# otaviog/align3d

Hardware: AMD Instinct MI355X
Metric: ICP frame-pairs/sec (640x480, 3-lvl, 15 iters) (higher is better)
Workload: dtype f32; 1 GPU; ms3x15 x 64 pairs/GPU, distinct frames, 640x480, 3 lvl x 15 it, HBM-resident (configs[4] shard); pairs_per_gpu=64, global_pairs=64, levels=3, distinct_frames=True, ranks_in_collective=1, collective=none

## Files before the change

### align3d_amd/csrc/image_icp.hip

```cpp
#include <cstdlib>
#include <memory>

#include "icp_engine.hpp"

using namespace a3d;

namespace {

struct LevelDesc {
  const float* src_points;
  const uint8_t* src_mask;
  const uint8_t* src_intensities;
  const float* tgt_points;
  const float* tgt_normals;
  const uint8_t* tgt_mask;
  const float* imap;
  uint32_t src_n;
  uint32_t tw, th;
  float fx, fy, cx, cy;
  uint32_t flags;
  uint32_t ppt;
  uint32_t src_w;
  const uint16_t* src_depth;
  const uint16_t* tgt_depth;
// ... 24 lines not shown
template <typename T>
__device__ __forceinline__ T ld(const void* base, uint32_t byte_off) {
  return *(const T __attribute__((address_space(1)))*)((gptr_c)base + byte_off);
}
typedef float f32x3 __attribute__((ext_vector_type(3)));
typedef f32x3 __attribute__((aligned(4))) f32x3_u;
typedef float f32x2 __attribute__((ext_vector_type(2)));
typedef f32x2 __attribute__((aligned(4))) f32x2_u;
__device__ __forceinline__ V3 ld_v3(const float* base, uint32_t idx) {
  uint32_t off;
  asm("v_lshl_add_u32 %0, %1, 1, %1" : "=v"(off) : "v"(idx));
  const f32x3 v = ld<f32x3_u>(base, off << 2);
  return {v.x, v.y, v.z};
}


__device__ __forceinline__ uint32_t texel_offset(uint32_t row, uint32_t width, uint32_t col) {
  return (__umul24(row, width) + col) * 4u;
}

__device__ __forceinline__ float bilerp(float v00, float v10, float v01, float v11, float uf, float vf) {
  float u0 = v00 * (1.0f - uf) + v10 * uf;
  float u1 = v01 * (1.0f - uf) + v11 * uf;
  return u0 * (1.0f - vf) + u1 * vf;
}
__device__ __forceinline__ float bilinear_at(const float* imap, uint32_t mw, float u, float v) {
  const uint32_t ui = f32_as_usize(u), vi = f32_as_usize(v);
  const uint32_t o = texel_offset(vi, mw, ui);
  const f32x2 a = ld<f32x2_u>(imap, o), b = ld<f32x2_u>(imap, o + mw * 4u);
  return bilerp(a.x, a.y, b.x, b.y, u - (float)ui, v - (float)vi);
}

struct SrcPx {
  V3 sp;
  uint8_t intensity;
  bool live;
  uint32_t depth, row, col;
};
struct BackProj {
  float fx, fy, cx, cy, scale;
  DivBy dfx, dfy;
};
struct BackProj2 {
  BackProj src, tgt;
};
__device__ __forceinline__ float uniform_f(float x) {
  return __int_as_float(__builtin_amdgcn_readfirstlane(__float_as_int(x)));
}
__device__ __forceinline__ BackProj make_backproj(const float (&k)[5]) {
  BackProj b;
  b.fx = k[0], b.fy = k[1], b.cx = k[2], b.cy = k[3], b.scale = k[4];
  const DivBy dx = div_prepare(b.fx), dy = div_prepare(b.fy);
  b.dfx = DivBy{uniform_f(dx.negz), uniform_f(dx.y)}, b.dfy = DivBy{uniform_f(dy.negz), uniform_f(dy.y)};
  return b;
}
constexpr int D16_TGT = 1, D16_SRC = 2;
#ifndef A3D_ICP_DEPTH16_SRC
#define A3D_ICP_DEPTH16_SRC 1
#endif
constexpr int D16_SIDES = D16_TGT | (A3D_ICP_DEPTH16_SRC ? D16_SRC : 0);
template <bool ZMASK = false, int D16 = 0>
__device__ __forceinline__ SrcPx stage_a(const LevelDesc& d, uint32_t i, bool in_range) {
  const uint32_t ii = in_range ? i : 0u;
  SrcPx s;
  if (D16 & D16_SRC) {
    const uint32_t r = f32_as_usize(((float)ii + 0.5f) * d.src_inv_w);
    s.row = r, s.col = ii - __umul24(r, d.src_w);
    s.depth = ld<uint16_t>(d.src_depth, ii * 2u);
    s.intensity = ld<uint8_t>(d.src_intensities, ii);
    s.live = in_range;
    return s;
  }
  s.sp = ld_v3(d.src_points, ii);
  s.intensity = ld<uint8_t>(d.src_intensities, ii);
  if (ZMASK) {
    s.live = in_range & (s.sp.z != 0.0f);
    return s;
  }
  const uint8_t mask = ld<uint8_t>(d.src_mask, ii);
  s.live = in_range & (mask != 0);
  return s;
}

struct ProjPx {
  V3 p;
  float u, v;
  V3 tp, tn;
  uint8_t tmask;
  bool live;
  uint32_t tdepth, trow, tcol;
};
template <bool ZMASK = false, int D16 = 0>
__device__ __forceinline__ ProjPx stage_b(const LevelDesc& d, const Pose& T, const SrcPx& s, float twf, float thf,
                                          const BackProj2& bp = BackProj2{}) {
  ProjPx o;
  V3 sp = s.sp;
  bool slive = s.live;
  if (D16 & D16_SRC) {
    sp = backproject_px_proven(s.depth, (int)s.row, (int)s.col, bp.src.cx, bp.src.cy, bp.src.scale, bp.src.dfx, bp.src.dfy);
    slive = slive & (s.depth != 0u);
  }
  o.p = transform_vector(T, sp);
  const float z = o.p.z, au = o.p.x * d.fx, av = o.p.y * d.fy;
  const DivBy dz = div_prepare(z);
  float qu = div_by(au, dz), qv = div_by(av, dz);
  if (__builtin_expect(__builtin_amdgcn_ballot_w64(!(div_den_ok(z) & div_num_ok(au) & div_num_ok(av))) != 0ull, 0))
    qu = au / z, qv = av / z;
  o.u = qu + d.cx;
  o.v = qv + d.cy;
  const float ur = o.u + 0.5f, vr = o.v + 0.5f;
  o.live = slive & !((ur <= -1.0f) | (ur >= twf) | (vr <= -1.0f) | (vr >= thf));
  const uint32_t col = (uint32_t)f32_as_i32(ur), row = (uint32_t)f32_as_i32(vr);
  const uint32_t tidx = o.live ? __umul24(row, d.tw) + col : 0u;
  if (D16 & D16_TGT) {
    o.tdepth = ld<uint16_t>(d.tgt_depth, tidx * 2u);
    o.trow = row, o.tcol = col;
    o.tn = ld_v3(d.tgt_normals, tidx);
    return o;
  }
  o.tp = ld_v3(d.tgt_points, tidx);
  o.tn = ld_v3(d.tgt_normals, tidx);
  o.tmask = ZMASK ? (uint8_t)0 : ld<uint8_t>(d.tgt_mask, tidx);
  return o;
}

struct MapPx {
  float t00, t10, t01, t11;
  uint32_t ui, vi;
};
template <bool ZMASK = false, int D16 = 0>
__device__ __forceinline__ MapPx stage_c(const LevelDesc& d, const Gates& gt, ProjPx& px, uint32_t mw,
                                         const BackProj2& bp = BackProj2{}) {
  bool tvalid;
  if (D16 & D16_TGT) {
    const uint32_t td = px.live ? px.tdepth : 0u;
    px.tp = backproject_px_proven(td, (int)px.trow, (int)px.tcol, bp.tgt.cx, bp.tgt.cy, bp.tgt.scale, bp.tgt.dfx, bp.tgt.dfy);
    tvalid = td != 0u;
  } else {
    tvalid = ZMASK ? px.tp.z != 0.0f : px.tmask == 1;
  }
  const V3 diff = px.tp - px.p;
  const float pn = dot(px.p, px.tn);
  px.live = px.live & tvalid
            & !(norm_squared(diff) > gt.max_distance_sqr)
            & !((pn >= -1.0f) & (pn <= gt.dot_reject_max));
  MapPx m;
  m.ui = f32_as_usize(px.u), m.vi = f32_as_usize(px.v);
  const uint32_t o = px.live ? texel_offset(m.vi, mw, m.ui) : 0u;
  const f32x2 a = ld<f32x2_u>(d.imap, o), b = ld<f32x2_u>(d.imap, o + mw * 4u);
  m.t00 = a.x, m.t10 = a.y, m.t01 = b.x, m.t11 = b.y;
  return m;
}

struct Terms {
  float Jg[6], rg;
  float Jc[6], rc;
  bool color;
};
template <bool EXACT = false>
__device__ __forceinline__ Terms stage_d(const LevelDesc& d, const Gates& gt, const ProjPx& px, const MapPx& m,
                                         uint8_t intensity, uint32_t mw) {
  auto fms = [](float a, float b, float c, float e) { return __builtin_fmaf(a, b, -(c * e)); };
  Terms t;
  const V3 P = px.p, n = px.tn;
  {
    const V3 df = px.tp - P;
    t.Jg[0] = n.x, t.Jg[1] = n.y, t.Jg[2] = n.z;
    if (EXACT) {
      t.rg = dot(df, n);
      const V3 tw = cross(P, n);
      t.Jg[3] = tw.x, t.Jg[4] = tw.y, t.Jg[5] = tw.z;
    } else {
      t.rg = __builtin_fmaf(df.z, n.z, __builtin_fmaf(df.y, n.y, df.x * n.x));
      t.Jg[3] = fms(P.y, n.z, P.z, n.y), t.Jg[4] = fms(P.z, n.x, P.x, n.z), t.Jg[5] = fms(P.x, n.y, P.y, n.x);
    }
  }
  const float uf = px.u - (float)m.ui, vf = px.v - (float)m.vi;
  const float value = bilerp(m.t00, m.t10, m.t01, m.t11, uf, vf);
  const float Hh = 0.005f, H_INV = 1.0f / 0.005f;
  const float u2 = px.u + Hh, v2 = px.v + Hh;
  float uh = bilerp(m.t00, m.t10, m.t01, m.t11, u2 - (float)m.ui, vf);
  float vh = bilerp(m.t00, m.t10, m.t01, m.t11, uf, v2 - (float)m.vi);
  const bool u_leaves = f32_as_usize(u2) != m.ui, v_leaves = f32_as_usize(v2) != m.vi;
  if (__builtin_expect(__builtin_amdgcn_ballot_w64(u_leaves | v_leaves) != 0ull, 0)) {
    if (u_leaves) uh = bilinear_at(d.imap, mw, u2, px.v);
    if (v_leaves) vh = bilinear_at(d.imap, mw, px.u, v2);
  }
  const float du = (uh - value) * H_INV;
  const float dv = (vh - value) * H_INV;
  const float sc = (float)intensity * 0.003921569f;
  const float z = P.z;
  t.rc = sc - value;
  t.color = t.rc * t.rc <= gt.max_color_distance_sqr;
  if (EXACT) {
    const float zz = z * z;
    const float dfx = d.fx / z, dcx = -P.x * d.fx / zz, dfy = d.fy / z, dcy = -P.y * d.fy / zz;
    const V3 gr{du * dfx, dv * dfy, du * dcx + dv * dcy};
    const V3 tw = cross(P, gr);
    t.Jc[0] = gr.x, t.Jc[1] = gr.y, t.Jc[2] = gr.z, t.Jc[3] = tw.x, t.Jc[4] = tw.y, t.Jc[5] = tw.z;
    return t;
  }
  const float r0 = __builtin_amdgcn_rcpf(z);
  const float rz = __builtin_fmaf(__builtin_fmaf(-z, r0, 1.0f), r0, r0), rzz = rz * rz;
  const float dfx = d.fx * rz, dfy = d.fy * rz, dcx = (-P.x * d.fx) * rzz, dcy = (-P.y * d.fy) * rzz;
  const V3 gr{du * dfx, dv * dfy, __builtin_fmaf(du, dcx, dv * dcy)};
  t.Jc[0] = gr.x, t.Jc[1] = gr.y, t.Jc[2] = gr.z;
  t.Jc[3] = fms(P.y, gr.z, P.z, gr.y), t.Jc[4] = fms(P.z, gr.x, P.x, gr.z), t.Jc[5] = fms(P.x, gr.y, P.y, gr.x);
  return t;
}

#ifdef A3D_DIAGNOSTICS
template <int G, bool MERGED>
__global__ void __launch_bounds__(256, MERGED ? 5 : 1)
    image_icp_kernel(const LevelDesc* __restrict__ descs, JobState* __restrict__ states, Gates gt,
                     float* __restrict__ partials, unsigned* __restrict__ counters, SolveArgs solve, int PPT) {
  const int pair = blockIdx.y;
  const uint32_t tile = blockIdx.x;
  constexpr int NACC = MERGED ? GN_MERGED : GN_PARTIAL;
  float acc[NACC];
#pragma unroll
  for (int k = 0; k < NACC; ++k) acc[k] = 0.0f;
  const float wg = solve.weight, wc = solve.color_weight;
  auto accumulate = [&](const Terms& t) {
    if (MERGED) {
      float Jg[6], Jc[6];
#pragma unroll
      for (int k = 0; k < 6; ++k) Jg[k] = wg * t.Jg[k], Jc[k] = t.color ? wc * t.Jc[k] : 0.0f;
      gn_step_merged(acc, t.rg, Jg, t.color ? t.rc : 0.0f, Jc, t.color ? 1.0f : 0.0f);
    } else {
      gn_step(acc, t.rg, t.Jg);
      if (t.color) gn_step(acc + (MERGED ? 0 : GN_ACC), t.rc, t.Jc);
    }
  };
  JobState* st = &states[pair];
// ... 38 lines not shown
    uint8_t cur_int[G];
#pragma unroll
    for (int g = 0; g < G; ++g) {
      const SrcPx s0 = src_at(0, g);
      s1[g] = src_at(G, g);
      cur[g] = stage_b(d, T, s0, twf, thf);
      cur_int[g] = s0.intensity;
    }
#pragma unroll 1
    for (int k0 = 0; k0 < PPT; k0 += G) {
      SrcPx s2[G];
      MapPx mp[G];
      ProjPx nxt[G];
      uint8_t nxt_int[G];
#pragma unroll
      for (int g = 0; g < G; ++g) s2[g] = src_at(k0 + 2 * G, g);
#pragma unroll
      for (int g = 0; g < G; ++g) mp[g] = stage_c(d, gt, cur[g], mw);
#pragma unroll
      for (int g = 0; g < G; ++g) {
        nxt[g] = stage_b(d, T, s1[g], twf, thf);
        nxt_int[g] = s1[g].intensity;
      }
#pragma unroll
      for (int g = 0; g < G; ++g) {
        if (cur[g].live) accumulate(stage_d(d, gt, cur[g], mp[g], cur_int[g], mw));
      }
#pragma unroll
      for (int g = 0; g < G; ++g) cur[g] = nxt[g], cur_int[g] = nxt_int[g], s1[g] = s2[g];
    }
    }
  }
#ifdef A3D_TAIL_STAMPS
  if (threadIdx.x == 0 && pair == 0 && blockIdx.x == 0) g_tail_stamps[9] = __builtin_amdgcn_s_memrealtime();
#endif
  SolveArgs sa = solve;
  if (st->status != A3D_OK) sa.mode = SOLVE_NONE;
  block_finish<NACC>(acc, partials + (size_t)pair * gridDim.x * GN_PARTIAL, tile, gridDim.x,
                     counters + pair, st, sa, pair);
}

__global__ void __launch_bounds__(256)
    image_icp_exact_kernel(const LevelDesc* __restrict__ descs, const JobState* __restrict__ states, Gates gt,
                           float* __restrict__ partials, int PPT) {
  float acc[GN_PARTIAL];
#pragma unroll
  for (int k = 0; k < GN_PARTIAL; ++k) acc[k] = 0.0f;
  const LevelDesc d = descs[0];
  const Pose T = states[0].pose;
  const uint32_t mw = d.tw + 2;
  const float twf = (float)d.tw, thf = (float)d.th;
  auto step_exact = [](float* a, float r, const float J[6]) {
    int t = 0;
    for (int i = 0; i < 6; ++i)
      for (int j = i; j < 6; ++j) {
        const float m = J[i] * J[j];
        a[t] = a[t] + m;
        ++t;
      }
    for (int i = 0; i < 6; ++i) {
      const float m = J[i] * r;
      a[21 + i] = a[21 + i] + m;
    }
    const float rr = r * r;
    a[27] = a[27] + rr;
    a[28] += 1.0f;
  };
  for (int k0 = 0; k0 < PPT; ++k0) {
    const uint32_t i = blockIdx.x * (256u * (uint32_t)PPT) + threadIdx.x + (uint32_t)k0 * 256u;
    const SrcPx s0 = stage_a(d, i, i < d.src_n);
    ProjPx px = stage_b(d, T, s0, twf, thf);
    const MapPx mp = stage_c(d, gt, px, mw);
    if (px.live) {
      const Terms t = stage_d<true>(d, gt, px, mp, s0.intensity, mw);
      step_exact(acc, t.rg, t.Jg);
      if (t.color) step_exact(acc + GN_ACC, t.rc, t.Jc);
    }
  }
  block_reduce_store<GN_PARTIAL, false>(acc, partials + (size_t)blockIdx.x * GN_PARTIAL);
}

#endif

template <bool ZMASK, int D16 = 0>
__device__ __forceinline__ SrcPx pixel_source_at(const LevelDesc& d, uint32_t base, int ppt, int k0) {
  const uint32_t i = base + (uint32_t)k0 * 256u;
  return stage_a<ZMASK, D16>(d, i, (k0 < ppt) && (i < d.src_n));
}
template <bool ZMASK, int D16 = 0>
__device__ __forceinline__ void pixel_pass(const LevelDesc& d, const Gates& gt, const Pose& T, uint32_t base, int ppt,
                                           const SrcPx& s0, SrcPx sa, float (&acc)[GN_PARTIAL]) {
  const uint32_t mw = d.tw + 2;
  const float twf = (float)d.tw, thf = (float)d.th;
  BackProj2 bp{};
  if (D16 & D16_SRC) bp.src = make_backproj(d.src_bp);
  if (D16 & D16_TGT) bp.tgt = make_backproj(d.tgt_bp);
  SrcPx sb;
  ProjPx pa = stage_b<ZMASK, D16>(d, T, s0, twf, thf, bp), pb;
  uint8_t ia = s0.intensity, ib;
  auto step = [&](ProjPx& cur, uint8_t cur_i, ProjPx& nxt, uint8_t& nxt_i, const SrcPx& s_next, SrcPx& s_new, int k0) {
    s_new = pixel_source_at<ZMASK, D16>(d, base, ppt, k0 + 2);
    if (D16) __builtin_amdgcn_sched_barrier(0);
    const MapPx mp = stage_c<ZMASK, D16>(d, gt, cur, mw, bp);
    nxt = stage_b<ZMASK, D16>(d, T, s_next, twf, thf, bp);
    nxt_i = s_next.intensity;
    if (cur.live) {
      const Terms t = stage_d(d, gt, cur, mp, cur_i, mw);
      gn_step(acc, t.rg, t.Jg);
      if (t.color) gn_step(acc + GN_ACC, t.rc, t.Jc);
    }
  };
#pragma unroll 1
  for (int k0 = 0; k0 < ppt; k0 += 2) {
    step(pa, ia, pb, ib, sa, sb, k0);
    step(pb, ib, pa, ia, sb, sa, k0 + 1);
  }
}

template <bool ZMASK, bool DEPTH16>
__global__ void __launch_bounds__(256, 1)
    image_icp_head_kernel(const LevelDesc* __restrict__ descs, const JobState* __restrict__ states_in,
                          JobState* __restrict__ states_out, Gates gt, const float* __restrict__ partials_in,
                          float* __restrict__ partials_out, uint32_t job_stride, HeadArgs head) {
  __shared__ uint32_t s_state[JOB_WORDS];
  const int pair = blockIdx.y;
  const uint32_t tile = blockIdx.x;
  float acc[GN_PARTIAL];
#pragma unroll
  for (int k = 0; k < GN_PARTIAL; ++k) acc[k] = 0.0f;
#if defined(A3D_DIAGNOSTICS) && defined(A3D_TAIL_STAMPS)
  const bool stamping = threadIdx.x == 0 && pair == 0 && tile + 1 == gridDim.x;
  unsigned long long* stamp = g_tail_stamps + 16 + 8 * ((states_out > states_in) ? 1 : 0);
#define A3D_HEAD_STAMP(k) do { if (stamping) stamp[k] = __builtin_amdgcn_s_memrealtime(); } while (0)
#else
#define A3D_HEAD_STAMP(k) do { } while (0)
#endif
  A3D_HEAD_STAMP(0);
  const LevelDesc d = descs[pair];
  const int ppt = (int)d.ppt;
  const uint32_t base = tile * (256u * (uint32_t)ppt) + threadIdx.x;
  constexpr int D16 = DEPTH16 ? D16_SIDES : 0;
  const SrcPx s0 = pixel_source_at<ZMASK, D16>(d, base, ppt, 0), s1 = pixel_source_at<ZMASK, D16>(d, base, ppt, 1);
  A3D_HEAD_STAMP(1);
  head_advance(states_in + pair, tile == 0 ? states_out + pair : nullptr, partials_in + (size_t)pair * job_stride, head,
               pair, s_state, tile == 0);
  A3D_HEAD_STAMP(2);
  if ((int)s_state[15] == A3D_OK) {
    auto uni = [&](int k) { return __uint_as_float(__builtin_amdgcn_readfirstlane(s_state[k])); };
    const Pose T{{uni(0), uni(1), uni(2)}, {uni(3), uni(4), uni(5), uni(6)}};
    pixel_pass<ZMASK, D16>(d, gt, T, base, ppt, s0, s1, acc);
  }
  A3D_HEAD_STAMP(3);
  block_reduce_store<GN_PARTIAL, false>(acc, partials_out + (size_t)pair * job_stride + (size_t)tile * GN_PARTIAL);
  A3D_HEAD_STAMP(4);
#undef A3D_HEAD_STAMP
}

#ifdef A3D_DIAGNOSTICS
struct PersistLevel {
  uint32_t desc_base;
  uint32_t iterations;
  uint32_t tiles;
  float weight, color_weight;
  Gates gates;
};
constexpr int PERSIST_MAX_LEVELS = 16;
constexpr uint32_t PAIR_CTRL_WORDS = 64;
constexpr uint32_t ROSTER_CLOSED = 0x80000000u;
constexpr unsigned long long ROSTER_WAIT_TICKS = 2000ull, PERSIST_SPIN_BOUND_TICKS = 200'000'000ull;
struct PersistPlan {
  uint32_t n_levels;
  uint32_t seq0;
  uint32_t counter_base;
  uint32_t finish;
  uint32_t parity;
  int trace_index0;
  int trace_stride;
  HeadArgs prev;
  PersistLevel lv[PERSIST_MAX_LEVELS];
};
struct PersistOut {
  Pose* poses;
  int32_t* status;
  float* matrices;
  unsigned long long* stamps;
};

template <bool ZMASK>
__global__ void __launch_bounds__(256, 4)
    image_icp_persistent_kernel(const LevelDesc* __restrict__ descs, uint32_t n_pairs_total, JobState* __restrict__ states,
                                float* __restrict__ partials, uint32_t partials_half, uint32_t job_stride,
                                unsigned* __restrict__ ctrl, PersistPlan plan, PersistOut out) {
  __shared__ uint32_t s_state[JOB_WORDS];
  __shared__ uint32_t s_rank, s_members;
  __shared__ int s_go;
  const int pair = blockIdx.y;
  unsigned* const counter = ctrl + (size_t)pair * PAIR_CTRL_WORDS;
  unsigned* const roster = counter + 1 + plan.parity;
  unsigned* const members = counter + 3 + plan.parity;
  float* const job_partials = partials + (size_t)pair * job_stride;
  if (threadIdx.x == 0) {
    const uint32_t old = __hip_atomic_fetch_add(roster, 1u, __ATOMIC_RELAXED, __HIP_MEMORY_SCOPE_AGENT);
    uint32_t rank = old & 0xffffu, R = 0;
    if (old & ROSTER_CLOSED) {
      rank = 0xffffffffu;
    } else {
      unsigned long long t0 = 0;
      for (uint32_t spin = 0;; ++spin) {
        R = __hip_atomic_load(members, __ATOMIC_RELAXED, __HIP_MEMORY_SCOPE_AGENT);
        if (R) break;
        uint32_t cur = __hip_atomic_load(roster, __ATOMIC_RELAXED, __HIP_MEMORY_SCOPE_AGENT);
        bool close = !(cur & ROSTER_CLOSED) && (cur & 0xffffu) >= gridDim.x;
        if (!close && !(cur & ROSTER_CLOSED) && (spin & 15u) == 15u) {
          const unsigned long long now = __builtin_amdgcn_s_memrealtime();
          if (!t0) t0 = now;
          close = now - t0 > ROSTER_WAIT_TICKS;
        }
        if (close && __hip_atomic_compare_exchange_strong(roster, &cur, cur | ROSTER_CLOSED, __ATOMIC_RELAXED,
                                                          __ATOMIC_RELAXED, __HIP_MEMORY_SCOPE_AGENT)) {
          R = cur & 0xffffu;
          __hip_atomic_store(members, R, __ATOMIC_RELAXED, __HIP_MEMORY_SCOPE_AGENT);
          break;
        }
        __builtin_amdgcn_s_sleep(1);
      }
    }
    s_rank = rank, s_members = R;
  }
  if (threadIdx.x < JOB_WORDS) s_state[threadIdx.x] = ((const uint32_t*)(states + (size_t)(plan.seq0 & 1u) * n_pairs_total + pair))[threadIdx.x];
  __syncthreads();
  const uint32_t rank = s_rank, R = s_members;
  if (rank == 0xffffffffu) return;
  HeadArgs prev = plan.prev;
  uint32_t seq = plan.seq0;
  uint32_t expected = plan.counter_base;
  int trace_index = plan.trace_index0;
  bool alive = true;
  auto head = [&](bool write_trace) {
    if (prev.mode != SOLVE_NONE) {
      if (threadIdx.x == 0) {
        int go = 1;
        unsigned long long t0 = 0;
        for (uint32_t spin = 0; (int)(__hip_atomic_load(counter, __ATOMIC_RELAXED, __HIP_MEMORY_SCOPE_AGENT) - expected) < 0; ++spin) {
          __builtin_amdgcn_s_sleep(1);
          if ((spin & 255u) == 255u) {
            const unsigned long long now = __builtin_amdgcn_s_memrealtime();
            if (!t0) t0 = now;
            if (now - t0 > PERSIST_SPIN_BOUND_TICKS) {
              go = 0;
              break;
            }
          }
        }
        s_go = go;
      }
      __syncthreads();
      if (!s_go) {
        alive = false;
        return;
      }
    }
    const uint32_t state_bits = threadIdx.x < JOB_WORDS ? s_state[threadIdx.x] : 0u;
    head_sum_and_advance<true>(state_bits, job_partials + (size_t)((seq + 1u) & 1u) * partials_half, prev, pair, s_state,
                               write_trace);
  };
#pragma unroll 1
  for (uint32_t l = 0; l < plan.n_levels && alive; ++l) {
    const PersistLevel lv = plan.lv[l];
    const LevelDesc d = descs[lv.desc_base + pair];
    const int ppt = (int)d.ppt;
    const uint32_t own_tiles = (d.src_n + 256u * d.ppt - 1u) / (256u * d.ppt);
    const uint32_t mine = rank < lv.tiles ? (lv.tiles - rank + R - 1u) / R : 0u;
    if (out.stamps && rank == 0 && threadIdx.x == 0) out.stamps[((size_t)pair * plan.n_levels + l) * 2] = __builtin_amdgcn_s_memrealtime();
#pragma unroll 1
    for (uint32_t it = 0; it < lv.iterations; ++it) {
      const uint32_t base0 = rank * (256u * (uint32_t)ppt) + threadIdx.x;
      SrcPx s0{}, s1{};
      if (mine) s0 = pixel_source_at<ZMASK, 0>(d, base0, ppt, 0), s1 = pixel_source_at<ZMASK, 0>(d, base0, ppt, 1);
      head(rank == 0);
      if (!alive) break;
      const bool ok = (int)s_state[15] == A3D_OK;
      auto uni = [&](int k) { return __uint_as_float(__builtin_amdgcn_readfirstlane(s_state[k])); };
      const Pose T{{uni(0), uni(1), uni(2)}, {uni(3), uni(4), uni(5), uni(6)}};
#pragma unroll 1
      for (uint32_t tile = rank; tile < lv.tiles; tile += R) {
        float acc[GN_PARTIAL];
#pragma unroll
        for (int k = 0; k < GN_PARTIAL; ++k) acc[k] = 0.0f;
        if (ok && tile < own_tiles) {
          const uint32_t base = tile * (256u * (uint32_t)ppt) + threadIdx.x;
          if (tile != rank) s0 = pixel_source_at<ZMASK, 0>(d, base, ppt, 0), s1 = pixel_source_at<ZMASK, 0>(d, base, ppt, 1);
          pixel_pass<ZMASK, 0>(d, lv.gates, T, base, ppt, s0, s1, acc);
        }
        block_reduce_store<GN_PARTIAL, true>(acc, job_partials + (size_t)(seq & 1u) * partials_half + (size_t)tile * GN_PARTIAL);
        __syncthreads();
      }
      if (mine) {
        asm volatile("s_waitcnt vmcnt(0)" ::: "memory");
        __syncthreads();
        if (threadIdx.x == 0) __hip_atomic_fetch_add(counter, mine, __ATOMIC_RELAXED, __HIP_MEMORY_SCOPE_AGENT);
      }
      expected += lv.tiles;
      prev.weight = lv.weight, prev.color_weight = lv.color_weight, prev.mode = SOLVE_IMAGE_ICP;
      prev.tiles = lv.tiles;
      prev.first_in_level = it == 0, prev.last_in_level = it + 1 == lv.iterations;
      prev.trace_index = trace_index++;
      ++seq;
    }
    if (out.stamps && rank == 0 && threadIdx.x == 0) out.stamps[((size_t)pair * plan.n_levels + l) * 2 + 1] = __builtin_amdgcn_s_memrealtime();
  }
  if (alive && plan.finish) head(rank == 0);
  if (rank != 0) return;
  if (threadIdx.x == 0) {
    __hip_atomic_store(counter + 1 + (plan.parity ^ 1u), 0u, __ATOMIC_RELAXED, __HIP_MEMORY_SCOPE_AGENT);
    __hip_atomic_store(counter + 3 + (plan.parity ^ 1u), 0u, __ATOMIC_RELAXED, __HIP_MEMORY_SCOPE_AGENT);
  }
  if (!alive) {
    if (threadIdx.x == 0) {
      states[(size_t)(seq & 1u) * n_pairs_total + pair].status = A3D_HIP_ERROR;
      if (out.status) out.status[pair] = A3D_HIP_ERROR;
    }
    return;
  }
  if (threadIdx.x < JOB_WORDS) ((uint32_t*)(states + (size_t)(seq & 1u) * n_pairs_total + pair))[threadIdx.x] = s_state[threadIdx.x];
  if (plan.finish && threadIdx.x == 0) {
    const float* f = (const float*)s_state;
    const Pose p{{f[0], f[1], f[2]}, {f[3], f[4], f[5], f[6]}};
    if (out.poses) out.poses[pair] = p;
    if (out.status) out.status[pair] = (int32_t)s_state[15];
    if (out.matrices) {
      float m[16];
      pose_to_matrix(p, m);
      for (int k = 0; k < 16; ++k) out.matrices[(size_t)pair * 16 + k] = m[k];
    }
  }
}

#endif

#ifdef A3D_DIAGNOSTICS
struct LevelPlan {
  uint32_t iterations;
  uint32_t epoch_base;
  int trace_base;
};

template <int G>
__global__ void __launch_bounds__(256, 3)
    image_icp_level_kernel(const LevelDesc* __restrict__ descs, JobState* __restrict__ states, Gates gt,
                           float* __restrict__ partials, unsigned* __restrict__ counters,
                           unsigned* __restrict__ epochs, SolveArgs solve, LevelPlan plan, int PPT) {
  __shared__ float s_pose[8];
  __shared__ int s_go;
  const int pair = blockIdx.y;
  JobState* st = &states[pair];
  const LevelDesc d = descs[pair];
  const uint32_t mw = d.tw + 2;
  const float twf = (float)d.tw, thf = (float)d.th;
  const uint32_t base = blockIdx.x * (256u * (uint32_t)PPT) + threadIdx.x;
  float* job_partials = partials + (size_t)pair * gridDim.x * GN_PARTIAL;
#pragma unroll 1
  for (uint32_t it = 0; it < plan.iterations; ++it) {
    if (threadIdx.x == 0) {
      const unsigned want = plan.epoch_base + it;
      int go = load_status(st) == A3D_OK;
      unsigned spins = 0;
      while (go && __hip_atomic_load(&epochs[pair], __ATOMIC_RELAXED, __HIP_MEMORY_SCOPE_AGENT) != want) {
        __builtin_amdgcn_s_sleep(4);
        ++spins;
        if ((spins & 63u) == 0 && load_status(st) != A3D_OK) go = 0;
        if (spins > (1u << 22)) {
          store_status(st, A3D_HIP_ERROR);
          go = 0;
        }
      }
// ... 354 lines not shown
    if (const char* env = getenv("A3D_ICP_GROUP_LEVELS")) {
      unsigned gl[3] = {1, 1, 1};
      sscanf(env, "%u,%u,%u", &gl[0], &gl[1], &gl[2]);
      if (l < 3) b->group[l] = (gl[l] == 2 || gl[l] == 4) ? gl[l] : 1;
    }
    if (const char* env = getenv("A3D_ICP_WAVES_LEVELS")) {
      float wl[3] = {waves, waves, waves};
      sscanf(env, "%f,%f,%f", &wl[0], &wl[1], &wl[2]);
      if (l < 3) w = wl[l];
    }
#endif
    uint32_t want = std::max(1u, (uint32_t)((float)b->resident_blocks * w / (float)P + 0.5f));
    if ((mask >> l) & 1u) want = std::min(want, persist_tiles_cap);
    if (pinned) want = pinned;
    uint32_t tiles = 0, ppt = 0;
    tiling_for(max_n, want, b->group[l], &tiles, &ppt);
#ifdef A3D_DIAGNOSTICS
    if (const char* env = getenv("A3D_ICP_VARIANT")) {
      unsigned ep = 0, eg = 0;
      if (sscanf(env, "%u,%u", &ep, &eg) == 2 && ep && (eg == 1 || eg == 2)) {
        b->group[l] = eg;
        ppt = ((ep + 1) / 2) * 2;
        tiles = (max_n + 256 * ppt - 1) / (256 * ppt);
      }
    }
#endif
    for (uint32_t p = 0; p < P; ++p) {
      LevelDesc& d = b->h_descs[(size_t)l * P + p];
      d.ppt = ppt;
      if (pinned) {
        uint32_t t_own = 0;
        tiling_for(d.src_n, pinned, 1, &t_own, &d.ppt);
        tiles = p == 0 ? t_own : std::max(tiles, t_own);
      }
    }
    b->tiles[l] = tiles, b->ppt[l] = ppt;
    if (((mask >> l) & 1u) && (uint64_t)tiles * P > b->persist_resident_blocks) mask &= ~(1u << l);
  }
  uint32_t run = 0;
  for (uint32_t l = L; l-- > 0;) {
    if (!((mask >> l) & 1u)) break;
    run |= 1u << l;
  }
  b->persist_mask = b->persist_disabled ? 0u : run;
}

#ifdef A3D_DIAGNOSTICS
a3d_status launch_pixel_kernel(a3d_multiscale_batch* b, uint32_t level, const SolveArgs& solve, uint32_t p0,
                               uint32_t count, hipStream_t s) {
  dim3 grid(b->tiles[level], count), block(256);
  const LevelDesc* descs = b->d_descs + (size_t)level * b->n_pairs + p0;
  JobState* states = b->d_states + p0;
  float* partials = b->d_partials + (size_t)p0 * b->max_tiles * GN_PARTIAL;
  unsigned* counters = b->d_counters + p0;
  const int ppt = (int)b->ppt[level];
  if (b->use_mfma) {
    if (b->group[level] == 2)
      hipLaunchKernelGGL((image_icp_mfma_kernel<2>), grid, block, 0, s, descs, states, b->gates[level],
                         partials, counters, solve, ppt);
    else
      hipLaunchKernelGGL((image_icp_mfma_kernel<1>), grid, block, 0, s, descs, states, b->gates[level],
                         partials, counters, solve, ppt);
  } else {
    if (b->group[level] == 4)
      hipLaunchKernelGGL((image_icp_kernel<4, false>), grid, block, 0, s, descs, states, b->gates[level], partials,
                         counters, solve, ppt);
    else if (b->group[level] == 2)
      hipLaunchKernelGGL((image_icp_kernel<2, false>), grid, block, 0, s, descs, states, b->gates[level], partials,
                         counters, solve, ppt);
    else if (b->merged_accumulators && solve.mode == SOLVE_IMAGE_ICP) {
      SolveArgs merged = solve;
      merged.mode = SOLVE_IMAGE_ICP_MERGED;
      hipLaunchKernelGGL((image_icp_kernel<1, true>), grid, block, 0, s, descs, states, b->gates[level], partials,
                         counters, merged, ppt);
    } else
      hipLaunchKernelGGL((image_icp_kernel<1, false>), grid, block, 0, s, descs, states, b->gates[level], partials,
                         counters, solve, ppt);
  }
  A3D_HIP_TRY(hipGetLastError());
  return A3D_OK;
}
#endif

a3d_status launch_head_kernel(a3d_multiscale_batch* b, uint32_t level, uint32_t seq, const HeadArgs& prev, uint32_t p0,
                              uint32_t count, hipStream_t s) {
  const uint32_t P = b->n_pairs;
  const uint32_t job_stride = b->max_tiles * GN_PARTIAL;
  const JobState* st_in = b->d_states + (size_t)(seq & 1u) * P + p0;
  JobState* st_out = b->d_states + (size_t)((seq + 1u) & 1u) * P + p0;
  const float* part_in = b->d_partials + (size_t)((seq + 1u) & 1u) * b->partials_half + (size_t)p0 * job_stride;
  float* part_out = b->d_partials + (size_t)(seq & 1u) * b->partials_half + (size_t)p0 * job_stride;
  const LevelDesc* descs = b->d_descs + (size_t)level * P + p0;
  if (b->depth16 && level == 0)
    hipLaunchKernelGGL((image_icp_head_kernel<true, true>), dim3(b->tiles[level], count), dim3(256), 0, s, descs, st_in,
                       st_out, b->gates[level], part_in, part_out, job_stride, prev);
  else if (b->zmask)
    hipLaunchKernelGGL((image_icp_head_kernel<true, false>), dim3(b->tiles[level], count), dim3(256), 0, s, descs, st_in,
                       st_out, b->gates[level], part_in, part_out, job_stride, prev);
  else
    hipLaunchKernelGGL((image_icp_head_kernel<false, false>), dim3(b->tiles[level], count), dim3(256), 0, s, descs, st_in,
                       st_out, b->gates[level], part_in, part_out, job_stride, prev);
  A3D_HIP_TRY(hipGetLastError());
  return A3D_OK;
}

a3d_status batch_commit_descs(a3d_multiscale_batch* b) {
  const uint32_t P = b->n_pairs, L = b->n_levels;
  plan_tiling(b);
  size_t max_partials = 1;
  for (uint32_t l = 0; l < L; ++l) max_partials = std::max(max_partials, (size_t)P * b->tiles[l] * GN_PARTIAL);
  b->max_tiles = (uint32_t)(max_partials / ((size_t)P * GN_PARTIAL));
  const char* zenv = A3D_DIAG_ENV("A3D_ICP_ZMASK");
  b->zmask = !(zenv && atoi(zenv) == 0);
  for (const LevelDesc& dsc : b->h_descs) b->zmask = b->zmask && (dsc.flags & 1u);
  const char* denv = A3D_DIAG_ENV("A3D_ICP_DEPTH16");
  b->depth16 = b->zmask && L > 0 && !(denv && atoi(denv) == 0);
  for (uint32_t p = 0; p < P && b->depth16; ++p) {
    const LevelDesc& dsc = b->h_descs[p];
    b->depth16 = (dsc.flags & 2u) && dsc.src_n <= (1u << 22);
  }
  b->partials_half = max_partials;
  if (b->partials_capacity < 2 * max_partials) {
    if (b->d_partials) A3D_HIP_TRY(hipFree(b->d_partials));
    b->d_partials = nullptr;
    b->partials_capacity = 0;
    A3D_HIP_TRY(hipMalloc((void**)&b->d_partials, 2 * max_partials * sizeof(float)));
    b->partials_capacity = 2 * max_partials;
  }
  A3D_HIP_TRY(hipMemcpyAsync(b->d_descs, b->h_descs.data(), b->h_descs.size() * sizeof(LevelDesc),
                             hipMemcpyHostToDevice, b->ctx->stream));
  return A3D_OK;
}

a3d_status batch_create(a3d_context* ctx, const a3d_icp_params* params, uint32_t n_levels, uint32_t n_pairs,
                        std::unique_ptr<a3d_multiscale_batch>* out) {
  auto b = std::make_unique<a3d_multiscale_batch>();
  b->ctx = ctx;
  b->n_pairs = n_pairs;
  b->n_levels = n_levels;
  b->params.assign(params, params + n_levels);
  for (uint32_t l = 0; l < n_levels; ++l) b->gates.push_back(make_gates(params[l]));
  b->tiles.assign(n_levels, 0);
  b->ppt.assign(n_levels, 2);
  b->group.assign(n_levels, 1);
  b->h_descs.resize((size_t)n_levels * n_pairs);
  auto resident = [&](auto kernel, int fallback_per_cu) {
    int per_cu = 0;
    if (hipOccupancyMaxActiveBlocksPerMultiprocessor(&per_cu, kernel, 256, 0) != hipSuccess || per_cu < 1)
      per_cu = fallback_per_cu;
    return (uint32_t)std::max(1, ctx->num_cus) * (uint32_t)std::max(0, per_cu);
  };
  b->resident_blocks = resident(image_icp_head_kernel<true, false>, 4);
#ifdef A3D_DIAGNOSTICS
  b->persist_resident_blocks = resident(image_icp_persistent_kernel<true>, 0);
  if (const char* env = getenv("A3D_ICP_ACCUM")) {
    b->use_mfma = strcmp(env, "mfma") == 0;
    b->merged_accumulators = strcmp(env, "merged") == 0;
  }
  if (const char* env = getenv("A3D_ICP_HANDOFF")) b->head_solve = strcmp(env, "ticket") != 0;
  if (const char* env = getenv("A3D_ICP_SOLVE")) b->exact_solve = strcmp(env, "exact") == 0;
  if (const char* env = getenv("A3D_ICP_PERSISTENT")) b->use_level_kernel = atoi(env) != 0;
  if (const char* env = getenv("A3D_ICP_PERSISTENT_LEVELS")) b->level_mask = (uint32_t)strtoul(env, nullptr, 0);
  if (!b->head_solve) b->resident_blocks = resident(image_icp_kernel<1, false>, 4);
  if (b->merged_accumulators) b->resident_blocks = resident(image_icp_kernel<1, true>, 4);
  b->level_resident_blocks = resident(image_icp_level_kernel<1>, 0);
  if (b->use_level_kernel && b->level_resident_blocks) b->resident_blocks = b->level_resident_blocks;
#endif
  A3D_HIP_TRY(hipSetDevice(ctx->device));
  {
    size_t total = 0;
    auto take = [&](size_t bytes) {
      const size_t at = total;
      total += ((bytes + 255) / 256) * 256;
      return at;
    };
    const size_t o_descs = take(b->h_descs.size() * sizeof(LevelDesc)), o_states = take(2 * n_pairs * sizeof(JobState)),
                 o_counters = take((size_t)n_pairs * CTRL_WORDS_PER_PAIR * sizeof(unsigned)), o_epochs = take(n_pairs * sizeof(unsigned)),
                 o_poses = take(n_pairs * sizeof(Pose)), o_init = take(n_pairs * sizeof(Pose)),
                 o_status = take(n_pairs * sizeof(int32_t)), o_readback = take(GN_PARTIAL * sizeof(double));
    A3D_HIP_TRY(hipMalloc((void**)&b->d_block, total));
    char* base = (char*)b->d_block;
    b->d_descs = (LevelDesc*)(base + o_descs), b->d_states = (JobState*)(base + o_states);
    b->d_counters = (unsigned*)(base + o_counters);
#ifdef A3D_DIAGNOSTICS
    b->d_epochs = (unsigned*)(base + o_epochs);
#else
    (void)o_epochs;
#endif
    b->d_poses = (Pose*)(base + o_poses), b->d_init = (Pose*)(base + o_init);
    b->d_status = (int32_t*)(base + o_status), b->d_readback = (double*)(base + o_readback);
  }
  if (CTRL_WORDS_PER_PAIR)
    A3D_HIP_TRY(hipMemsetAsync(b->d_counters, 0, (size_t)n_pairs * CTRL_WORDS_PER_PAIR * sizeof(unsigned), ctx->stream));
  b->n_streams = n_pairs >= 12 ? 3u : (n_pairs >= 8 ? 2u : 1u);
  if (const char* env = A3D_DIAG_ENV("A3D_ICP_STREAMS")) b->n_streams = (uint32_t)std::min(4, std::max(1, atoi(env)));
  b->n_streams = std::min(b->n_streams, n_pairs);
#ifdef A3D_DIAGNOSTICS
  if (b->use_level_kernel) b->n_streams = 1u;
#endif
  if (b->n_streams > 1) {
    A3D_HIP_TRY(hipEventCreateWithFlags(&b->ev_fork, hipEventDisableTiming));
    for (uint32_t g = 1; g < b->n_streams; ++g) {
      A3D_TRY(ctx_side_stream(ctx, g - 1, &b->aux_streams[g - 1]));
      A3D_HIP_TRY(hipEventCreateWithFlags(&b->ev_join[g - 1], hipEventDisableTiming));
    }
  }
  A3D_HIP_TRY(hipEventCreate(&b->ev0));
  A3D_HIP_TRY(hipEventCreate(&b->ev1));
  *out = std::move(b);
  return A3D_OK;
}

a3d_status batch_enqueue(a3d_multiscale_batch* b, const Pose* d_init, uint32_t levels_to_run, float* d_matrices,
                         float* d_trace, int trace_stride) {
  hipStream_t s = b->ctx->stream;
  const uint32_t P = b->n_pairs;
  b->last_init = d_init, b->last_levels = levels_to_run, b->last_matrices = d_matrices;
  b->persist_used = false;
  A3D_HIP_TRY(hipEventRecord(b->ev0, s));
  A3D_TRY(launch_job_init(s, b->d_states, d_init, (int)P));
  size_t kidx = 0;
  int trace_index = 0;
  auto profile_begin = [&](hipStream_t ps) -> a3d_status {
    if (!b->profile_kernels) return A3D_OK;
    if (b->kev.size() < 2 * (kidx + 1)) {
      hipEvent_t e0, e1;
      A3D_HIP_TRY(hipEventCreate(&e0));
      A3D_HIP_TRY(hipEventCreate(&e1));
      b->kev.push_back(e0);
      b->kev.push_back(e1);
    }
    A3D_HIP_TRY(hipEventRecord(b->kev[2 * kidx], ps));
    return A3D_OK;
  };
  uint32_t profile_level = 0;
// ... 682 lines not shown
```

Before: 24610 frame-pairs/s.

## Issue intensity-map loads early in projection stage and add deeper pipeline option

The bilinear intensity-map loads move from the correspondence-check stage into the projection stage, so they are in flight one pipeline step earlier. Loads are now gated only by the projection bounds, not by the full rejection tests, so some of them are wasted. It also adds an optional three-deep software pipeline that parks projected points in shared memory to limit register pressure. The default is the early-map form (PIPE_MAP), and the deep form can be selected under diagnostics.

```diff
diff --git a/align3d_amd/csrc/image_icp.hip b/align3d_amd/csrc/image_icp.hip
--- a/align3d_amd/csrc/image_icp.hip
+++ b/align3d_amd/csrc/image_icp.hip
@@ -130,6 +130,19 @@
   return s;
 }
 
+struct MapPx {
+  float t00, t10, t01, t11;
+  uint32_t ui, vi;
+};
+__device__ __forceinline__ MapPx map_cell_request(const float* imap, uint32_t mw, float u, float v, bool inside) {
+  MapPx m;
+  m.ui = f32_as_usize(u), m.vi = f32_as_usize(v);
+  const uint32_t o = inside ? texel_offset(m.vi, mw, m.ui) : 0u;
+  const f32x2 a = ld<f32x2_u>(imap, o), b = ld<f32x2_u>(imap, o + mw * 4u);
+  m.t00 = a.x, m.t10 = a.y, m.t01 = b.x, m.t11 = b.y;
+  return m;
+}
+
 struct ProjPx {
   V3 p;
   float u, v;
@@ -137,10 +150,11 @@
   uint8_t tmask;
   bool live;
   uint32_t tdepth, trow, tcol;
+  MapPx map;
 };
-template <bool ZMASK = false, int D16 = 0>
+template <bool ZMASK = false, int D16 = 0, bool EARLY_MAP = false>
 __device__ __forceinline__ ProjPx stage_b(const LevelDesc& d, const Pose& T, const SrcPx& s, float twf, float thf,
-                                          const BackProj2& bp = BackProj2{}) {
+                                          const BackProj2& bp = BackProj2{}, uint32_t mw = 0) {
   ProjPx o;
   V3 sp = s.sp;
   bool slive = s.live;
@@ -164,19 +178,17 @@
     o.tdepth = ld<uint16_t>(d.tgt_depth, tidx * 2u);
     o.trow = row, o.tcol = col;
     o.tn = ld_v3(d.tgt_normals, tidx);
+    if (EARLY_MAP) o.map = map_cell_request(d.imap, mw, o.u, o.v, o.live);
     return o;
   }
   o.tp = ld_v3(d.tgt_points, tidx);
   o.tn = ld_v3(d.tgt_normals, tidx);
   o.tmask = ZMASK ? (uint8_t)0 : ld<uint8_t>(d.tgt_mask, tidx);
+  if (EARLY_MAP) o.map = map_cell_request(d.imap, mw, o.u, o.v, o.live);
   return o;
 }
 
-struct MapPx {
-  float t00, t10, t01, t11;
-  uint32_t ui, vi;
-};
-template <bool ZMASK = false, int D16 = 0>
+template <bool ZMASK = false, int D16 = 0, bool EARLY_MAP = false>
 __device__ __forceinline__ MapPx stage_c(const LevelDesc& d, const Gates& gt, ProjPx& px, uint32_t mw,
                                          const BackProj2& bp = BackProj2{}) {
   bool tvalid;
@@ -192,12 +204,13 @@
   px.live = px.live & tvalid
             & !(norm_squared(diff) > gt.max_distance_sqr)
             & !((pn >= -1.0f) & (pn <= gt.dot_reject_max));
-  MapPx m;
-  m.ui = f32_as_usize(px.u), m.vi = f32_as_usize(px.v);
-  const uint32_t o = px.live ? texel_offset(m.vi, mw, m.ui) : 0u;
-  const f32x2 a = ld<f32x2_u>(d.imap, o), b = ld<f32x2_u>(d.imap, o + mw * 4u);
-  m.t00 = a.x, m.t10 = a.y, m.t01 = b.x, m.t11 = b.y;
-  return m;
+  if (EARLY_MAP) {
+    MapPx m = px.map;
+    asm volatile("v_cvt_u32_f32_e32 %0, %1" : "=v"(m.ui) : "v"(px.u));
+    asm volatile("v_cvt_u32_f32_e32 %0, %1" : "=v"(m.vi) : "v"(px.v));
+    return m;
+  }
+  return map_cell_request(d.imap, mw, px.u, px.v, px.live);
 }
 
 struct Terms {
@@ -402,34 +415,67 @@
 
 #endif
 
+constexpr int PIPE_PARENT = 0, PIPE_MAP = 1, PIPE_DEEP = 2;
 template <bool ZMASK, int D16 = 0>
 __device__ __forceinline__ SrcPx pixel_source_at(const LevelDesc& d, uint32_t base, int ppt, int k0) {
   const uint32_t i = base + (uint32_t)k0 * 256u;
   return stage_a<ZMASK, D16>(d, i, (k0 < ppt) && (i < d.src_n));
 }
-template <bool ZMASK, int D16 = 0>
+template <bool ZMASK, int D16 = 0, int PIPE = PIPE_PARENT>
 __device__ __forceinline__ void pixel_pass(const LevelDesc& d, const Gates& gt, const Pose& T, uint32_t base, int ppt,
-                                           const SrcPx& s0, SrcPx sa, float (&acc)[GN_PARTIAL]) {
+                                           const SrcPx& s0, SrcPx sa, SrcPx sb, float (&acc)[GN_PARTIAL]) {
+  constexpr bool EARLY = PIPE != PIPE_PARENT;
+  constexpr int AHEAD = PIPE == PIPE_DEEP ? 3 : 2;
   const uint32_t mw = d.tw + 2;
   const float twf = (float)d.tw, thf = (float)d.th;
   BackProj2 bp{};
   if (D16 & D16_SRC) bp.src = make_backproj(d.src_bp);
   if (D16 & D16_TGT) bp.tgt = make_backproj(d.tgt_bp);
-  SrcPx sb;
-  ProjPx pa = stage_b<ZMASK, D16>(d, T, s0, twf, thf, bp), pb;
-  uint8_t ia = s0.intensity, ib;
-  auto step = [&](ProjPx& cur, uint8_t cur_i, ProjPx& nxt, uint8_t& nxt_i, const SrcPx& s_next, SrcPx& s_new, int k0) {
-    s_new = pixel_source_at<ZMASK, D16>(d, base, ppt, k0 + 2);
+  __shared__ float s_park[PIPE == PIPE_DEEP ? 3 * 5 * 256 : 1];
+  auto park = [&](int slot, const ProjPx& px) {
+    float* q = s_park + slot * (5 * 256) + threadIdx.x;
+    q[0] = px.p.x, q[256] = px.p.y, q[512] = px.p.z, q[768] = px.u, q[1024] = px.v;
+  };
+  auto unpark = [&](int slot, ProjPx& px) {
+    const float* q = s_park + slot * (5 * 256) + threadIdx.x;
+    px.p = V3{q[0], q[256], q[512]}, px.u = q[768], px.v = q[1024];
+  };
+  auto step = [&](ProjPx& cur, uint8_t cur_i, ProjPx& nxt, uint8_t& nxt_i, const SrcPx& s_next, SrcPx& s_new, int k0,
+                  int cur_slot = 0, int nxt_slot = 0) {
+    if (PIPE == PIPE_DEEP) unpark(cur_slot, cur);
+    s_new = pixel_source_at<ZMASK, D16>(d, base, ppt, k0 + AHEAD);
     if (D16) __builtin_amdgcn_sched_barrier(0);
-    const MapPx mp = stage_c<ZMASK, D16>(d, gt, cur, mw, bp);
-    nxt = stage_b<ZMASK, D16>(d, T, s_next, twf, thf, bp);
+    const MapPx mp = stage_c<ZMASK, D16, EARLY>(d, gt, cur, mw, bp);
+    nxt = stage_b<ZMASK, D16, EARLY>(d, T, s_next, twf, thf, bp, mw);
     nxt_i = s_next.intensity;
+    if (PIPE == PIPE_DEEP) park(nxt_slot, nxt);
     if (cur.live) {
       const Terms t = stage_d(d, gt, cur, mp, cur_i, mw);
       gn_step(acc, t.rg, t.Jg);
       if (t.color) gn_step(acc + GN_ACC, t.rc, t.Jc);
     }
   };
+  ProjPx pa = stage_b<ZMASK, D16, EARLY>(d, T, s0, twf, thf, bp, mw), pb;
+  uint8_t ia = s0.intensity, ib;
+  if (PIPE == PIPE_DEEP) {
+    ProjPx pc;
+    uint8_t ic;
+    pb = stage_b<ZMASK, D16, EARLY>(d, T, sa, twf, thf, bp, mw), ib = sa.intensity;
+    park(0, pa), park(1, pb);
+#pragma unroll 1
+    for (int k0 = 0;; k0 += 6) {
+      step(pa, ia, pc, ic, sb, sa, k0, 0, 2);
+      step(pb, ib, pa, ia, sa, sb, k0 + 1, 1, 0);
+      if (k0 + 2 >= ppt) break;
+      step(pc, ic, pb, ib, sb, sa, k0 + 2, 2, 1);
+      step(pa, ia, pc, ic, sa, sb, k0 + 3, 0, 2);
+      if (k0 + 4 >= ppt) break;
+      step(pb, ib, pa, ia, sb, sa, k0 + 4, 1, 0);
+      step(pc, ic, pb, ib, sa, sb, k0 + 5, 2, 1);
+      if (k0 + 6 >= ppt) break;
+    }
+    return;
+  }
 #pragma unroll 1
   for (int k0 = 0; k0 < ppt; k0 += 2) {
     step(pa, ia, pb, ib, sa, sb, k0);
@@ -437,7 +483,7 @@
   }
 }
 
-template <bool ZMASK, bool DEPTH16>
+template <bool ZMASK, bool DEPTH16, int PIPE>
 __global__ void __launch_bounds__(256, 1)
     image_icp_head_kernel(const LevelDesc* __restrict__ descs, const JobState* __restrict__ states_in,
                           JobState* __restrict__ states_out, Gates gt, const float* __restrict__ partials_in,
@@ -461,6 +507,8 @@
   const uint32_t base = tile * (256u * (uint32_t)ppt) + threadIdx.x;
   constexpr int D16 = DEPTH16 ? D16_SIDES : 0;
   const SrcPx s0 = pixel_source_at<ZMASK, D16>(d, base, ppt, 0), s1 = pixel_source_at<ZMASK, D16>(d, base, ppt, 1);
+  SrcPx s2{};
+  if (PIPE == PIPE_DEEP) s2 = pixel_source_at<ZMASK, D16>(d, base, ppt, 2);
   A3D_HEAD_STAMP(1);
   head_advance(states_in + pair, tile == 0 ? states_out + pair : nullptr, partials_in + (size_t)pair * job_stride, head,
                pair, s_state, tile == 0);
@@ -468,7 +516,7 @@
   if ((int)s_state[15] == A3D_OK) {
     auto uni = [&](int k) { return __uint_as_float(__builtin_amdgcn_readfirstlane(s_state[k])); };
     const Pose T{{uni(0), uni(1), uni(2)}, {uni(3), uni(4), uni(5), uni(6)}};
-    pixel_pass<ZMASK, D16>(d, gt, T, base, ppt, s0, s1, acc);
+    pixel_pass<ZMASK, D16, PIPE>(d, gt, T, base, ppt, s0, s1, s2, acc);
   }
   A3D_HEAD_STAMP(3);
   block_reduce_store<GN_PARTIAL, false>(acc, partials_out + (size_t)pair * job_stride + (size_t)tile * GN_PARTIAL);
@@ -610,7 +658,7 @@
         if (ok && tile < own_tiles) {
           const uint32_t base = tile * (256u * (uint32_t)ppt) + threadIdx.x;
           if (tile != rank) s0 = pixel_source_at<ZMASK, 0>(d, base, ppt, 0), s1 = pixel_source_at<ZMASK, 0>(d, base, ppt, 1);
-          pixel_pass<ZMASK, 0>(d, lv.gates, T, base, ppt, s0, s1, acc);
+          pixel_pass<ZMASK, 0>(d, lv.gates, T, base, ppt, s0, s1, SrcPx{}, acc);
         }
         block_reduce_store<GN_PARTIAL, true>(acc, job_partials + (size_t)(seq & 1u) * partials_half + (size_t)tile * GN_PARTIAL);
         __syncthreads();
@@ -1131,6 +1179,23 @@
 }
 #endif
 
+#ifndef A3D_ICP_PIPE_DEFAULT
+#define A3D_ICP_PIPE_DEFAULT 1
+#endif
+constexpr int PIPE_DEFAULT = A3D_ICP_PIPE_DEFAULT;
+#ifdef A3D_DIAGNOSTICS
+int head_pipe_form(const a3d_multiscale_batch* b, uint32_t level) {
+  int form = PIPE_DEFAULT;
+  if (const char* env = getenv("A3D_ICP_PIPE")) {
+    int pl[3] = {-1, -1, -1};
+    const int n = sscanf(env, "%d,%d,%d", &pl[0], &pl[1], &pl[2]);
+    const int v = n == 1 ? pl[0] : (level < 3 ? pl[level] : -1);
+    if (v >= PIPE_PARENT && v <= PIPE_DEEP) form = v;
+  }
+  return form;
+}
+#endif
+
 a3d_status launch_head_kernel(a3d_multiscale_batch* b, uint32_t level, uint32_t seq, const HeadArgs& prev, uint32_t p0,
                               uint32_t count, hipStream_t s) {
   const uint32_t P = b->n_pairs;
@@ -1140,15 +1205,28 @@
   const float* part_in = b->d_partials + (size_t)((seq + 1u) & 1u) * b->partials_half + (size_t)p0 * job_stride;
   float* part_out = b->d_partials + (size_t)(seq & 1u) * b->partials_half + (size_t)p0 * job_stride;
   const LevelDesc* descs = b->d_descs + (size_t)level * P + p0;
-  if (b->depth16 && level == 0)
-    hipLaunchKernelGGL((image_icp_head_kernel<true, true>), dim3(b->tiles[level], count), dim3(256), 0, s, descs, st_in,
-                       st_out, b->gates[level], part_in, part_out, job_stride, prev);
-  else if (b->zmask)
-    hipLaunchKernelGGL((image_icp_head_kernel<true, false>), dim3(b->tiles[level], count), dim3(256), 0, s, descs, st_in,
-                       st_out, b->gates[level], part_in, part_out, job_stride, prev);
-  else
-    hipLaunchKernelGGL((image_icp_head_kernel<false, false>), dim3(b->tiles[level], count), dim3(256), 0, s, descs, st_in,
-                       st_out, b->gates[level], part_in, part_out, job_stride, prev);
+  const dim3 grid(b->tiles[level], count);
+#define A3D_HEAD_LAUNCH(ZM, D16, PIPE)                                                                                  \
+  hipLaunchKernelGGL((image_icp_head_kernel<ZM, D16, PIPE>), grid, dim3(256), 0, s, descs, st_in, st_out, b->gates[level], \
+                     part_in, part_out, job_stride, prev)
+  const bool d16 = b->depth16 && level == 0;
+#define A3D_HEAD_LAUNCH_FORM(PIPE)                             \
+  do {                                                         \
+    if (d16) A3D_HEAD_LAUNCH(true, true, PIPE);                \
+    else if (b->zmask) A3D_HEAD_LAUNCH(true, false, PIPE);     \
+    else A3D_HEAD_LAUNCH(false, false, PIPE);                  \
+  } while (0)
+#ifdef A3D_DIAGNOSTICS
+  switch (head_pipe_form(b, level)) {
+    case PIPE_PARENT: A3D_HEAD_LAUNCH_FORM(PIPE_PARENT); break;
+    case PIPE_MAP: A3D_HEAD_LAUNCH_FORM(PIPE_MAP); break;
+    default: A3D_HEAD_LAUNCH_FORM(PIPE_DEEP); break;
+  }
+#else
+  A3D_HEAD_LAUNCH_FORM(PIPE_DEFAULT);
+#endif
+#undef A3D_HEAD_LAUNCH_FORM
+#undef A3D_HEAD_LAUNCH
   A3D_HIP_TRY(hipGetLastError());
   return A3D_OK;
 }
@@ -1199,7 +1277,7 @@
       per_cu = fallback_per_cu;
     return (uint32_t)std::max(1, ctx->num_cus) * (uint32_t)std::max(0, per_cu);
   };
-  b->resident_blocks = resident(image_icp_head_kernel<true, false>, 4);
+  b->resident_blocks = resident(image_icp_head_kernel<true, false, PIPE_DEFAULT>, 4);
 #ifdef A3D_DIAGNOSTICS
   b->persist_resident_blocks = resident(image_icp_persistent_kernel<true>, 0);
   if (const char* env = getenv("A3D_ICP_ACCUM")) {
```

Result: faster. 25010 frame-pairs/s (median of 6 runs) (+1.6%).
